# etlundquist/robot-ebert

Measured on AMD Instinct MI355X. Metric: queries/sec + top-K index match, 1M×d=1536 batch=4096, at 1/2/4/8 MI355X, higher is better.
Workload: dtype f64

## Files before the change

include/ebert.h:

```cpp
#ifndef EBERT_H_
#define EBERT_H_

#include <stddef.h>
#include <stdint.h>

#ifdef __cplusplus
extern "C" {
#endif

#define EBT_OK 0
#define EBT_EINVAL (-1)
#define EBT_EHIP (-2)
#define EBT_ENOMEM (-3)
#define EBT_EUNSUPPORTED (-4)

#define EBT_F32 0
#define EBT_BF16 1
#define EBT_F16 2
#define EBT_F64 3

int ebt_version(void);

const char* ebt_last_error(void);

// ... 58 lines not shown
size_t ebt_sort_exclusions_bytes(int64_t B, int64_t nnz);
int ebt_sort_exclusions(const int64_t* off, const int64_t* rows_in, int64_t* rows_out, int64_t B,
                        int64_t nnz, void* workspace, size_t ws_bytes, void* stream);

int ebt_merge_topk(const double* scores, const int64_t* rows, int32_t R, int64_t B, int32_t k,
                   double* out_scores, int64_t* out_rows, void* stream);

int64_t ebt_shard_list_width(int32_t k, int32_t world);
int64_t ebt_shard_sample_tiles(int64_t n_global, int32_t world, int64_t B_pad);
int64_t ebt_shard_pack_cap(int64_t B, int32_t k, int32_t world, int64_t n_global);
size_t ebt_shard_pack_bytes(int64_t B, int64_t cap);
int ebt_shard_pack(const double* scores, const int64_t* rows, int64_t B, int32_t k,
                   const double* t_floor, int64_t cap, void* send, void* stream);
int ebt_merge_packed(const void* recv, int32_t R, int64_t B, int32_t k, int64_t cap,
                     double* out_scores, int64_t* out_rows, int32_t* incomplete, void* stream);

int ebt_screen_exact(const double* q64, int64_t B, int32_t d, const void* cat, int dtype,
                     int64_t ld, const double* gnorm64, int64_t n_rows, float* scores,
                     int64_t ld_scores, void* stream);

#define EBT_FLAG_NO_FUSE 1
#define EBT_FLAG_EXACT 2
#define EBT_FLAG_THETA 4
#define EBT_EXACT_EPS 1.1920928955078125e-07f
int ebt_cosine_topk_plan(int64_t B, int64_t B_pad, int64_t n_rows, int32_t kprime,
                         int64_t chunk_rows, int flags, int64_t* head_rows, int64_t* cap,
                         int64_t* chunk, int32_t* fused);
int ebt_cosine_topk_spec_plan(int64_t B, int64_t B_pad, int64_t n_rows, int32_t kprime,
                              int flags, int64_t* sample_tiles, int64_t* tile_stride,
                              int32_t* rank, double* hits);
int64_t ebt_cosine_topk_spec_lead(int64_t B, int64_t B_pad, int64_t n_rows, int32_t kprime,
                                  int flags);
int ebt_spec_lead(int on);
size_t ebt_cosine_topk_workspace(int64_t B, int64_t B_pad, int64_t n_rows, int32_t kprime,
                                 int64_t chunk_rows, int flags);

int ebt_cosine_topk_prepared(const double* q64, const void* qimg, const float* qscale, const float* eps,
                    int64_t B, int64_t B_pad, const void* cat, int dtype, int64_t ld,
                    const double* gnorm64, const void* cimg, const float* cscale, int img_dtype,
                    int32_t ld_img, int64_t n_rows, int32_t d, int32_t d_pad, int64_t row_offset,
                    const int64_t* excl_off, const int64_t* excl_rows, int32_t k, int32_t kprime,
                    int64_t chunk_rows, int flags, void* workspace, size_t ws_bytes,
                    double* out_scores, int64_t* out_rows, int32_t* certified, void* timer,
                    void* stream);

typedef struct ebt_catalog {
  const void* data;
  int32_t dtype, d;
  int64_t n, ld, row_offset;
  double* gnorm64;
  float* inv32;
  const void* image;
  const float* cscale;
  int32_t img_dtype, ld_img, d_pad, native;
  float u_cat;
} ebt_catalog;

size_t ebt_catalog_state_bytes(const void* data, int dtype, int64_t n, int32_t d, int64_t ld);
int ebt_catalog_init(ebt_catalog* cat, const void* data, int dtype, int64_t n, int32_t d,
                     int64_t ld, int64_t row_offset, void* state, size_t state_bytes,
                     void* stream);

int ebt_catalog_init_reserved(ebt_catalog* cat, const void* data, int dtype, int64_t n,
                              int64_t n_cap, int32_t d, int64_t ld, int64_t row_offset,
                              void* state, size_t state_bytes, void* stream);

// ... 338 lines not shown
```

robot_ebert_amd/_lib.py:

```python
from __future__ import annotations

import ctypes
import os
import threading
from typing import Optional

import torch

_HERE = os.path.dirname(os.path.abspath(__file__))
LIB_PATH = os.environ.get("EBERT_LIB", os.path.join(_HERE, "libebert.so"))

EBT_F32, EBT_BF16, EBT_F16, EBT_F64 = 0, 1, 2, 3
DTYPE_CODE = {torch.float32: EBT_F32, torch.bfloat16: EBT_BF16, torch.float16: EBT_F16,
              torch.float64: EBT_F64}
STAGES = {"gemm": 0, "mask": 1, "select": 2, "merge_select": 3, "rescore": 4, "gemm_filter": 5,
          "prep": 6, "shard_merge": 7, "collective_wait": 8, "small": 9}
EBT_FLAG_NO_FUSE = 1
EBT_FLAG_EXACT = 2
EBT_FLAG_THETA = 4
EBT_FLAG_LIKED_CHECKED = 8
EBT_FILTER_SLOTS_MAX = 128
EBT_EXPLAIN_M_MAX = 64
EBT_MMR_POOL_MAX = 512
EBT_INTEREST_MAX = 8
# ... 186 lines not shown
    "ebt_cosine_sample_lead": ([_VP, _VP, _I64, _VP, _VP, _INT, _I32, _I64, _I32, _I64, _I64,
                                _VP, _I64, _I64, _VP, _I64, _VP, _VP], _INT),
    "ebt_cosine_screen_at_lead": ([_VP, _VP, _VP, _VP, _I64, _I64, _VP, _INT, _I64, _VP, _VP,
                                   _VP, _INT, _I32, _I64, _I32, _I32, _I64, _VP, _VP, _I32,
                                   _I32, _I64, _INT, _VP, ctypes.c_size_t, _VP, _VP, _VP, _VP,
                                   _VP, ctypes.c_double, _I64, _VP, _I64, _VP, _VP], _INT),
    "ebt_pool_kth": ([_VP, _I64, _I64, _I64, _I32, _I32, _VP, _VP], _INT),
    "ebt_union_floor": ([_VP, _I32, _I64, _I32, _I32, _VP, _VP], _INT),
    "ebt_certify_cut": ([_VP, _VP, _VP, _VP, _VP, _I64, _VP], _INT),
    "ebt_rescore_owned": ([_VP, _I64, _I32, _VP, _INT, _I64, _VP, _I64, _I64, _VP, _VP, _I32,
                           _I32, _VP, _VP, _VP], _INT),
    "ebt_finalize_topk": ([_VP, _VP, _VP, _I64, _I32, _I32, _I64, _VP, _VP, _VP, _VP, _VP, _VP],
                          _INT),
    "ebt_merge_hits": ([_VP, _VP, _I64, _I32, _I32, _VP, _I64, _I32, _VP, _I64, _I64, _I64, _VP, _VP, _VP,
                        _VP], _INT),
    "ebt_mask_excluded": ([_VP, _I64, _I64, _I64, _I64, _VP, _VP, _VP], _INT),
    "ebt_select_topk": ([_VP, _VP, _I64, _I64, _I64, _I64, _I32, _I32, _VP, _VP, _I64, _VP],
                        _INT),
    "ebt_rescore": ([_VP, _I64, _I32, _VP, _INT, _I64, _VP, _I64, _VP, _VP, _I32, _I32, _I64, _VP,
                     _VP, _VP, _VP, _VP, _VP, _VP], _INT),
    "ebt_rescore_form": ([_INT], _INT),
    "ebt_wave_sum_check": ([_VP, _I64, _VP, _VP, _VP], _INT),
    "ebt_sort_exclusions_bytes": ([_I64, _I64], _SZ),
    "ebt_sort_exclusions": ([_VP, _VP, _VP, _I64, _I64, _VP, _SZ, _VP], _INT),
    "ebt_merge_topk": ([_VP, _VP, _I32, _I64, _I32, _VP, _VP, _VP], _INT),
    "ebt_screen_exact": ([_VP, _I64, _I32, _VP, _INT, _I64, _VP, _I64, _VP, _I64, _VP], _INT),
    "ebt_cosine_topk_workspace": ([_I64, _I64, _I64, _I32, _I64, _INT], _SZ),
    "ebt_cosine_topk_plan": ([_I64, _I64, _I64, _I32, _I64, _INT, ctypes.POINTER(_I64),
                              ctypes.POINTER(_I64), ctypes.POINTER(_I64),
                              ctypes.POINTER(ctypes.c_int32)], _INT),
    "ebt_cosine_topk_spec_plan": ([_I64, _I64, _I64, _I32, _INT, ctypes.POINTER(_I64),
                                   ctypes.POINTER(_I64), ctypes.POINTER(ctypes.c_int32),
                                   ctypes.POINTER(ctypes.c_double)], _INT),
    "ebt_cosine_topk_prepared": ([_VP, _VP, _VP, _VP, _I64, _I64, _VP, _INT, _I64, _VP, _VP, _VP, _INT,
                         _I32, _I64, _I32, _I32, _I64, _VP, _VP, _I32, _I32, _I64, _INT, _VP, _SZ,
                         _VP, _VP, _VP, _VP, _VP], _INT),
    "ebt_als_gram": ([_VP, _I64, _I32, _VP, _VP], _INT),
    "ebt_als_solve": ([_VP, _VP, _I32, _I64, _VP, _VP, _VP, _F32, _F32, _VP, _VP], _INT),
    "ebt_timer_create": ([], _VP),
    "ebt_timer_destroy": ([_VP], None),
    "ebt_timer_reset": ([_VP], _INT),
    "ebt_timer_set_mask": ([_VP, ctypes.c_uint32], _INT),
    "ebt_timer_query": ([_VP, _INT, ctypes.POINTER(ctypes.c_double), ctypes.POINTER(_I64)], _INT),
    "ebt_timer_begin": ([_VP, _INT, _VP], _INT),
    "ebt_timer_end": ([_VP, _INT, _VP], _INT),
    "ebt_timer_count_rows": ([_VP, _INT], _INT),
    "ebt_timer_rows": ([_VP, ctypes.POINTER(_I64)], _INT),
}

_lib: Optional[ctypes.CDLL] = None
_lock = threading.Lock()


def load() -> ctypes.CDLL:
    global _lib
    if _lib is not None:
        return _lib
    with _lock:
        if _lib is None:
            if not os.path.exists(LIB_PATH):
                raise EbertError(
                    f"{LIB_PATH} not found: build it with `python -c 'import __graft_entry__ as g; "
                    "g.build()'` (make -C robot_ebert_amd/csrc)")
            try:
                lib = ctypes.CDLL(LIB_PATH)
            except OSError as e:
# ... 94 lines not shown
```

robot_ebert_amd/csrc/api.hip:

```cpp
#include <atomic>
#include <cstdarg>
#include <cstdlib>
#include <cstdio>
#include <cstring>
#include <mutex>
#include <vector>

#include "common.h"
#include "internal.h"

namespace ebt {

static thread_local char g_err[512] = "";

void set_error(const char* fmt, ...) {
  va_list ap;
  va_start(ap, fmt);
  vsnprintf(g_err, sizeof(g_err), fmt, ap);
  va_end(ap);
}

int hip_check(hipError_t e, const char* what) {
  if (e == hipSuccess) return EBT_OK;
  set_error("%s: %s", what, hipGetErrorString(e));
// ... 374 lines not shown
  if (selects && L.segs > 1) o = align_up(o + (size_t)B * L.segs * kprime * 4);
  L.off_segi = o;
  if (selects && L.segs > 1) o = align_up(o + (size_t)B * L.segs * kprime * 8);
  L.off_chv = o;
  if (selects && L.n_chunks > 1) o = align_up(o + (size_t)B * L.n_chunks * kprime * 4);
  L.off_chi = o;
  if (selects && L.n_chunks > 1) o = align_up(o + (size_t)B * L.n_chunks * kprime * 8);
  L.off_fv = o;
  o = align_up(o + (size_t)B * kprime * 4);
  L.off_fi = o;
  o = align_up(o + (size_t)B * kprime * 8);
  if (L.fused) {
    L.off_cand = o;
    o = align_up(o + (size_t)B_pad * L.ld_cand * 8);
    L.off_counts = o;
    o = align_up(o + (size_t)B_pad * L.ld_counts);
    L.off_thr = o;
    o = align_up(o + (size_t)B_pad * 4);
    L.off_ovf = o;
    o = align_up(o + (size_t)B_pad * 4);
  }
  L.off_eps = o;
  if (flags & EBT_FLAG_EXACT) o = align_up(o + (size_t)B_pad * 4);
  if (L.spec) {
    L.off_tspec = o;
    o = align_up(o + (size_t)B_pad * 4);
  }
  L.off_lead = o;
  if (L.ld_lead) o = align_up(o + (size_t)B_pad * L.ld_lead * 4);
  L.bytes = o;
  return L;
}

static int head_topk(const PipeArgs& a, const WsLayout& L, char* ws, int64_t r0, int64_t nrows,
                     float* dv_final, int64_t* di_final, int64_t ld_final, void* timer,
                     hipStream_t st) {
  const QueryOps& q = a.q;
  const CatOps& c = a.c;
  const int64_t B = q.B, row_offset = c.row_offset;
  const int32_t kprime = a.kprime;
  const bool exact = a.flags & EBT_FLAG_EXACT;
  float* S = (float*)(ws + L.off_s);
  float* segv = (float*)(ws + L.off_segv);
  int64_t* segi = (int64_t*)(ws + L.off_segi);
  float* chv = (float*)(ws + L.off_chv);
  int64_t* chi = (int64_t*)(ws + L.off_chi);
  const int64_t n_chunks = ceil_div(nrows, L.chunk);
  int rc;
  for (int64_t ch = 0; ch < n_chunks; ++ch) {
    const int64_t c0 = r0 + ch * L.chunk;
    const int64_t nc = (r0 + nrows - c0) < L.chunk ? (r0 + nrows - c0) : L.chunk;
    {
      StageScope s(timer, EBT_STAGE_GEMM, st);
      if (exact) {
        rc = screen_exact(q.q64, B, c.d, (const char*)c.cat + c0 * c.ld * dtype_size(c.dtype),
                          c.dtype, c.ld,
                          c.gnorm64 + c0, nc, S, L.ld_s, st);
      } else {
        rc = screen_gemm(q.qimg, q.B_pad, (const char*)c.cimg + c0 * c.ld_img * 2, nc, c.d_pad,
                         c.ld_img, c.img_dtype, q.qscale, c.cscale ? c.cscale + c0 : nullptr, S,
                         L.ld_s, st);
      }
    }
    if (rc) return rc;
    if (a.excl.off || a.allow) {
      StageScope s(timer, EBT_STAGE_MASK, st);
// ... 14 lines not shown
      } else {
        rc = select_topk(S, nullptr, L.ld_s, B, nc, c0, kprime, L.segs, segv, segi,
                         (int64_t)L.segs * kprime, st);
        if (!rc)
          rc = select_topk(segv, segi, (int64_t)L.segs * kprime, B, (int64_t)L.segs * kprime, 0,
                           kprime, 1, dv, di, ld_d, st);
      }
    }
    if (rc) return rc;
  }
  if (n_chunks > 1) {
    StageScope s(timer, EBT_STAGE_MERGE_SELECT, st);
    rc = select_topk(chv, chi, n_chunks * kprime, B, n_chunks * kprime, 0, kprime, 1, dv_final,
                     di_final, ld_final, st);
    if (rc) return rc;
  }
  return EBT_OK;
}

int rescore_sharded(const double* q64, int64_t B, const CatOps& c, const CandList& l, int32_t k,
                    const float* eps, const double* t_floor, double* out_s, int64_t* out_r,
                    int32_t* certified, RescoreExtras x, void* timer, hipStream_t st) {
  StageScope sc(timer, EBT_STAGE_RESCORE, st);
  x.gathered = timer_rows(timer, st);
  return rescore(q64, B, c, l, k, eps, t_floor, out_s, out_r, certified, x, st);
}

}

using namespace ebt;

extern "C" {

int ebt_version(void) { return 1200; }

const char* ebt_last_error(void) { return g_err; }

int ebt_row_norms(const void* x, int dtype, int64_t n, int32_t d, int64_t ld, double* gnorm64,
                  float* inv32, void* stream) {
  return row_norms(x, dtype, n, d, ld, gnorm64, inv32, (hipStream_t)stream);
}

int ebt_screen_image(const void* x, int dtype, int64_t n, int32_t d, int64_t ld,
                     const double* gnorm64, int normalize, int img_dtype, void* img,
                     int32_t ld_img, void* stream) {
  return screen_image(x, dtype, n, d, ld, gnorm64, normalize, img_dtype, img, ld_img,
                      (hipStream_t)stream);
}

int ebt_query_dense(const void* q, int dtype, int64_t B, int32_t d, int64_t ldq, double* q64,
                    void* stream) {
  return query_dense(q, dtype, B, d, ldq, q64, (hipStream_t)stream);
}

int ebt_query_liked_sum(const void* cat, int dtype, int32_t d, int64_t ld,
                        const double* gnorm64_cat, int64_t B, const int64_t* liked_off,
                        const int64_t* liked_rows, double* q64, void* stream) {
  return query_liked_sum(cat, dtype, d, ld, gnorm64_cat, B, liked_off, liked_rows, q64,
                         (hipStream_t)stream, 0, 0);
}

int ebt_query_liked_wsum(const void* cat, int dtype, int32_t d, int64_t ld,
                         const double* gnorm64_cat, int64_t B, const int64_t* liked_off,
                         const int64_t* liked_rows, const double* liked_w, double* q64,
                         void* stream) {
  return query_liked_wsum(cat, dtype, d, ld, gnorm64_cat, B, liked_off, liked_rows, liked_w, q64,
                          (hipStream_t)stream, 0, 0);
// ... 116 lines not shown
    return EBT_EINVAL;
  }
  const WsLayout L = ws_layout(B, B_pad, n_rows, kprime, chunk_rows, flags);
  *head_rows = L.head;
  *cap = L.fused ? L.seg_max : 0;
  *chunk = L.chunk;
  *fused = L.fused ? 1 : 0;
  return EBT_OK;
}

int ebt_cosine_topk_spec_plan(int64_t B, int64_t B_pad, int64_t n_rows, int32_t kprime,
                              int flags, int64_t* sample_tiles, int64_t* tile_stride,
                              int32_t* rank, double* hits) {
  if (B < 0 || B_pad < B || n_rows < 1 || kprime < 1 || !sample_tiles || !tile_stride || !rank ||
      !hits) {
    set_error("ebt_cosine_topk_spec_plan: bad arguments");
    return EBT_EINVAL;
  }
  const WsLayout L = ws_layout(B, B_pad, n_rows, kprime, 1024, flags);
  *sample_tiles = L.spec ? L.spec_tiles : 0;
  *tile_stride = L.spec ? L.spec_stride : 0;
  *rank = L.spec ? L.spec_j : 0;
  *hits = L.spec ? L.spec_hits : 0.0;
  return EBT_OK;
}

int64_t ebt_cosine_topk_spec_lead(int64_t B, int64_t B_pad, int64_t n_rows, int32_t kprime,
                                  int flags) {
  if (B < 0 || B_pad < B || n_rows < 1 || kprime < 1) return -1;
  const WsLayout L = ws_layout(B, B_pad, n_rows, kprime, 1024, flags);
  return L.spec ? L.spec_lead : 0;
}

int ebt_spec_lead(int on) {
  if (on < 0) return spec_lead_flag().load();
  return spec_lead_flag().exchange(on != 0 ? 1 : 0);
}

}

namespace ebt {
namespace {

struct ScreenOut {
  float* fv;
  int64_t* fi;
  const float* eps;
  const int* ovf;
  const float* theta;
};

}

static int check_pipe(const PipeArgs& a, const char* who) {
  const QueryOps& q = a.q;
  const CatOps& c = a.c;
  const bool exact = a.flags & EBT_FLAG_EXACT;
  if (!q.q64 || (!exact && (!q.qimg || !q.qscale || !q.eps || !c.cimg)) || !c.cat ||
      !c.gnorm64) {
    set_error("%s: null pointer", who);
    return EBT_EINVAL;
  }
  if (q.B < 1 || q.B_pad < q.B || q.B_pad % 128 != 0 || c.n_rows < 1 || c.d < 1 ||
      c.d_pad < c.d || c.d_pad % 64 != 0 || c.ld_img < c.d_pad || a.k < 1 || a.kprime < a.k ||
      a.kprime > 4096 || a.kprime % 4 != 0 || a.chunk_rows < 128 || a.chunk_rows % 128 != 0 ||
      ((a.excl.off == nullptr) != (a.excl.rows == nullptr))) {
    set_error("%s: bad arguments (B=%lld B_pad=%lld n=%lld d=%d d_pad=%d k=%d kprime=%d "
              "chunk=%lld)", who, (long long)q.B, (long long)q.B_pad, (long long)c.n_rows, c.d,
              c.d_pad, a.k, a.kprime, (long long)a.chunk_rows);
    return EBT_EINVAL;
  }
  return EBT_OK;
}

static int filter_screen(const PipeArgs& a, int64_t r0, int64_t seg, const float* thr,
                         const HitSlots& h, int* ovf, void* timer, hipStream_t st) {
  const QueryOps& q = a.q;
  const CatOps& c = a.c;
  const int64_t part = filter_split_rows(q.B_pad, seg);
  const int64_t step = part > 0 ? part : seg;
  for (int64_t p0 = 0; p0 < seg; p0 += step) {
    const int64_t nr = seg - p0 < step ? seg - p0 : step;
    const int64_t r = r0 + p0;
    const HitSlots hp = from_group(h, p0 / 256);
    KernelStage s(timer, EBT_STAGE_GEMM_FILTER, st);
    const int rc = screen_gemm_filter(q.qimg, q.B_pad, (const char*)c.cimg + r * c.ld_img * 2, nr,
                                      c.d_pad, c.ld_img, c.img_dtype, q.qscale,
                                      c.cscale ? c.cscale + r : nullptr, thr, hp.cand, hp.ld_cand,
                                      hp.slots, hp.counts, hp.ld_counts, ovf, r, st);
    if (rc) return rc;
  }
  return EBT_OK;
}

static int run_screen_spec(const PipeArgs& a, const WsLayout& L, char* ws, float* fv,
                           int64_t* fi, void* timer, hipStream_t st) {
  int rc;
  const QueryOps& q = a.q;
  const CatOps& c = a.c;
  const int64_t B = q.B, B_pad = q.B_pad, n_rows = c.n_rows;
  const int32_t k = a.k, kprime = a.kprime;
  float* thr = (float*)(ws + L.off_thr);
  int* ovf = (int*)(ws + L.off_ovf);
  float* pooled = (float*)(ws + L.off_s);
  float* tspec = (float*)(ws + L.off_tspec);
  const int64_t m = L.head;
  const bool given = a.theta != nullptr || a.gsamp != nullptr;
  const double spec_hits = given ? (a.hits > 0.0 ? a.hits : 1.0) : L.spec_hits;
  const double per_group = spec_hits * (double)L.group_rows / (double)n_rows;
  const double n_cells = (double)B * (double)ceil_div(n_rows, L.group_rows);
  int slots = 8;
  while (slots < EBT_FILTER_SLOTS_MAX &&
         (slots < 4.0 * per_group + 4.0 || n_cells * poisson_tail(1.5 * per_group, slots) > 1e-3))
    slots *= 2;
  const HitSlots h{(uint64_t*)(ws + L.off_cand), L.ld_cand, slots, (uint8_t*)(ws + L.off_counts),
                   L.ld_counts};
  float* own_lead = (float*)(ws + L.off_lead);
  const LeadIn li = given ? a.lead : LeadIn{own_lead, L.ld_lead, L.spec_lead};
  const int64_t lead = li.tiles;
  if (lead > 0 && (lead * slots > L.ld_cand || lead > L.ld_counts || L.group_rows != 256)) {
    set_error("run_screen_spec: the lead does not fit the hit slots");
    return EBT_EINVAL;
  }
  if (given) {
    if (a.gsamp)
      rc = pool_kth(a.gsamp, a.gs_G, B, B_pad, a.gs_G, a.gs_j, tspec, fv, fi, kprime, ovf, li, h,
                    a.gs, st);
    else
      rc = spec_given_init(a.theta, B, B_pad, tspec, fv, fi, kprime, ovf, li, h, st);
    if (rc) return rc;
  } else {
    {
      StageScope s(timer, EBT_STAGE_GEMM, st);
      rc = screen_gemm_pool(q.qimg, B_pad, c.cimg, m, c.d_pad, c.ld_img, c.img_dtype, q.qscale,
                            c.cscale, 256 * L.spec_stride, pooled, L.ld_s, st, lead, own_lead,
                            L.ld_lead);
    }
    if (rc) return rc;
    {
      StageScope s(timer, EBT_STAGE_SELECT, st);
      rc = pool_kth(pooled, L.ld_s, B, B_pad, (int)(m / 64), L.spec_j, tspec, fv, fi, kprime, ovf,
                    li, h, {}, st);
    }
    if (rc) return rc;
  }
  const bool wave = merge_wave_fits(kprime);
  int64_t seg_cap = L.ld_cand / slots;
  const int64_t max_groups = wave ? merge_wave_max_groups() : merge_block_max_groups(kprime);
  seg_cap = seg_cap < max_groups ? seg_cap : max_groups;
  seg_cap *= L.group_rows;
  const double cap = (double)(wave ? merge_wave_capacity() : merge_block_capacity(kprime));
  double f_spread = 2.5;
  if (!given && L.spec_j > 0) {
    const double target = 1e-2 / (double)(B > 0 ? B : 1);
    double x = (double)L.spec_j;
    while (x < 8.0 * L.spec_j) {
      double pmf = exp(-x), cdf = pmf;
      for (int i = 1; i < L.spec_j; ++i) {
        pmf *= x / i;
        cdf += pmf;
      }
      if (cdf <= target) break;
      x += 0.25;
    }
    f_spread = x / (double)L.spec_j;
    f_spread = f_spread < 2.5 ? 2.5 : f_spread;
  }
  int64_t r0 = 256 * lead;
  bool first = true, verified = false, thr_raised = false;
  while (r0 < n_rows) {
    const int64_t g0 = first ? lead : 0;
    const int64_t cap_rows = seg_cap - g0 * L.group_rows;
    const double room = (cap - kprime) / f_spread;
    const double kept = 0.5 * ((double)k + (double)kprime);
    double rate = spec_hits / (double)n_rows;
    if (!first && kept / (double)r0 < rate) rate = kept / (double)r0;
    int64_t seg = (int64_t)(room / (rate > 1e-12 ? rate : 1e-12));
    seg = (seg + 255) / 256 * 256;
    if (L.round_rows > 0 && seg >= L.round_rows) seg = seg / L.round_rows * L.round_rows;
    seg = seg < 256 ? 256 : seg;
    const int64_t cap_r = L.round_rows > 0 && cap_rows >= L.round_rows
                              ? cap_rows / L.round_rows * L.round_rows : cap_rows;
    seg = seg < cap_r ? seg : cap_r;
    if (!first && n_rows - r0 - seg < seg / 2) seg = n_rows - r0;
    if (seg > cap_rows) seg = cap_rows;
    if (seg > n_rows - r0) seg = n_rows - r0;
    if (seg < 1) {
      set_error("run_screen_spec: no room for a segment");
      return EBT_EINVAL;
    }
    const float* t = tspec;
    if (!first) {
      if (!thr_raised) {
        rc = spec_threshold(fv, kprime, B, B_pad, k, q.eps, tspec, thr, ovf, 0, st);
        if (rc) return rc;
      }
      t = thr;
    }
    rc = filter_screen(a, r0, seg, t, from_group(h, g0), ovf, timer, st);
    if (rc) return rc;
    const bool fuse_verify = wave && !given && r0 + seg == n_rows;
    verified |= fuse_verify;
    const int64_t groups = g0 + ceil_div(seg, L.group_rows);
    const bool last = r0 + seg == n_rows;
    thr_raised = wave && !last;
    {
      StageScope s(timer, EBT_STAGE_MERGE_SELECT, st);
      if (wave) {
        WaveMergeOpts o{};
        if (fuse_verify) o.verify = {tspec, q.eps};
        if (last && a.floor_out) o.floor = {a.floor_out, a.floor_w, q.eps};
        if (thr_raised) o.raise = {thr, tspec, q.eps, B_pad};
        rc = merge_segment_wave(fv, fi, B, kprime, k, h, groups, c.row_offset, a.excl, ovf, st, o);
      } else {
        rc = merge_segment(fv, fi, B, kprime, h, groups, c.row_offset, a.excl, ovf, st,
                           rate * (double)(seg + g0 * L.group_rows));
      }
    }
    if (rc) return rc;
    r0 += seg;
    first = false;
  }
  if (given || verified) return EBT_OK;
  return spec_threshold(fv, kprime, B, B_pad, k, q.eps, tspec, nullptr, ovf, 1, st);
}

static int run_screen(const PipeArgs& a, const WsLayout& L, char* ws, float* fv, int64_t* fi,
                      void* timer, hipStream_t st, ScreenOut* so) {
  int rc;
  const QueryOps& q = a.q;
  const CatOps& c = a.c;
  so->eps = q.eps;
  so->ovf = nullptr;
  const int64_t B = q.B, B_pad = q.B_pad, n_rows = c.n_rows, row_offset = c.row_offset;
  const int32_t k = a.k, kprime = a.kprime;
  if (a.flags & EBT_FLAG_EXACT) {
    float* xeps = (float*)(ws + L.off_eps);
    const float e = EBT_EXACT_EPS;
    uint32_t bits;
    memcpy(&bits, &e, 4);
    rc = hip_check(hipMemsetD32Async((hipDeviceptr_t)xeps, (int)bits, (size_t)B, st),
                   "hipMemsetD32Async");
    if (rc) return rc;
    so->eps = xeps;
    return head_topk(a, L, ws, 0, n_rows, fv, fi, kprime, timer, st);
  }
  if (!L.fused) return head_topk(a, L, ws, 0, n_rows, fv, fi, kprime, timer, st);
  float* thr = (float*)(ws + L.off_thr);
// ... 427 lines not shown
```

robot_ebert_amd/csrc/internal.h:

```cpp
#pragma once

#include "common.h"

namespace ebt {

struct QueryOps {
  const double* q64;
  const void* qimg;
  const float *qscale, *eps;
  int64_t B, B_pad;
};
struct CatOps {
  const void* cat; int dtype; int64_t ld; const double* gnorm64;
  const void* cimg; const float* cscale; int img_dtype; int32_t ld_img;
  int64_t n_rows; int32_t d, d_pad; int64_t row_offset;
};
inline CatOps cat_ops(const ebt_catalog& c) {
  return {c.data, c.dtype, c.ld, c.gnorm64, c.image, c.cscale, c.img_dtype, c.ld_img, c.n, c.d,
          c.d_pad, c.row_offset};
}
struct ExclCsr { const int64_t *off, *rows; };
struct HitSlots {
  uint64_t* cand; int64_t ld_cand; int slots;
  uint8_t* counts; int64_t ld_counts;
// ... 26 lines not shown
struct RescoreExtras {
  const int* ovf; const float* theta; ExclCsr excl;
  const ShardPackOut* pack; unsigned long long* gathered;
};

int64_t shard_lead_room(int64_t B_pad, int64_t n_rows, int64_t sample_tiles);
int64_t shard_lead_tiles(int64_t B_pad, int64_t n_rows, int64_t sample_tiles);
int rescore_sharded(const double* q64, int64_t B, const CatOps& c, const CandList& l, int32_t k,
                    const float* eps, const double* t_floor, double* out_s, int64_t* out_r,
                    int32_t* certified, RescoreExtras x, void* timer, hipStream_t st);
int topk_prepared(const PipeArgs& a, void* workspace, size_t ws_bytes, double* out_scores,
                  int64_t* out_rows, int32_t* certified, void* timer, hipStream_t st);
int screen_export(const PipeArgs& a, void* workspace, size_t ws_bytes, float* list_vals,
                  int64_t* list_rows, int32_t* ovf_out, float* eps_out, void* timer,
                  hipStream_t st);
int screen_at_local(const PipeArgs& a, void* workspace, size_t ws_bytes, float* list_vals,
                    int64_t* list_rows, const float** theta_dev, const int** ovf_dev,
                    const float** eps_dev, void* timer, hipStream_t st);

int64_t gemm_cus();
int screen_gemm(const void* qimg, int64_t B_pad, const void* cimg, int64_t n_rows, int32_t d_pad,
                int32_t ld_img, int img_dtype, const float* qscale, const float* cscale,
                float* scores, int64_t ld_scores, hipStream_t stream, int64_t cstride = 0);
int screen_gemm_pool(const void* qimg, int64_t B_pad, const void* cimg, int64_t n_rows,
                     int32_t d_pad, int32_t ld_img, int img_dtype, const float* qscale,
                     const float* cscale, int64_t cstride, float* pooled, int64_t ld_pooled,
                     hipStream_t stream, int64_t lead, float* lead_scores, int64_t ld_lead);
int64_t filter_group_rows(int64_t B_pad);
int screen_gemm_filter(const void* qimg, int64_t B_pad, const void* cimg, int64_t n_rows,
                       int32_t d_pad, int32_t ld_img, int img_dtype, const float* qscale,
                       const float* cscale, const float* thr, uint64_t* cand, int64_t ld_cand,
                       int slots, uint8_t* counts, int64_t ld_counts, int* ovf, int64_t idx_base,
                       hipStream_t stream);
int64_t filter_split_rows(int64_t B_pad, int64_t n_rows);

int select_topk(const float* vals, const int64_t* idx, int64_t ld, int64_t B, int64_t n,
                int64_t idx_base, int32_t kprime, int32_t segs, float* out_vals, int64_t* out_idx,
                int64_t ld_out, hipStream_t stream);
int merge_segment(float* fv, int64_t* fi, int64_t B, int kprime, const HitSlots& h,
                  int64_t n_groups, int64_t row_offset, const ExclCsr& excl, int* ovf,
                  hipStream_t st, double expect_hits = 0.0);
bool merge_wave_fits(int kprime);
int merge_block_capacity(int kprime);
int64_t merge_block_max_groups(int kprime);
int64_t merge_wave_max_groups();
int merge_wave_capacity();
int merge_segment_wave(float* fv, int64_t* fi, int64_t B, int kprime, int k, const HitSlots& h,
                       int64_t n_groups, int64_t row_offset, const ExclCsr& excl, int* ovf,
                       hipStream_t st, const WaveMergeOpts& o = {});
int pilot_topk(const float* S, int64_t ld_s, int64_t B, int n, int64_t idx_base, int kprime, int k,
               float* fv, int64_t* fi, hipStream_t st);
int kth_threshold(const float* vals, int64_t ld, int64_t B, int64_t B_pad, int k, const float* eps,
                  float* thr, hipStream_t st);
int pool_kth(const float* pool, int64_t ld, int64_t B, int64_t B_pad, int G, int j, float* thr,
             float* fv, int64_t* fi, int kprime, int* ovf, const LeadIn& lead, const HitSlots& h,
             const GatheredSamples& gs, hipStream_t st);
int spec_given_init(const float* theta, int64_t B, int64_t B_pad, float* tspec, float* fv,
                    int64_t* fi, int kprime, int* ovf, const LeadIn& lead, const HitSlots& h,
                    hipStream_t st);
int spec_threshold(const float* vals, int64_t ld, int64_t B, int64_t B_pad, int k,
                   const float* eps, const float* thr_spec, float* thr, int* ovf, int mode,
                   hipStream_t st);

int row_norms(const void* x, int dtype, int64_t n, int32_t d, int64_t ld, double* gnorm,
              float* inv32, hipStream_t st);
int screen_image(const void* x, int dtype, int64_t n, int32_t d, int64_t ld, const double* gnorm,
                 int normalize, int img_dtype, void* img, int32_t ld_img, hipStream_t st,
// ... 55 lines not shown
```

robot_ebert_amd/csrc/screen_gemm.hip:

```cpp
#include <hip/hip_ext.h>

#include <atomic>
#include <cstdlib>
#include <type_traits>

#include "common.h"
#include "internal.h"

namespace ebt {

constexpr int GBM = 128;
constexpr int GBN = 128;
constexpr int GBK = 64;
constexpr int GTHREADS = 256;
constexpr int GTILE_BYTES = GBM * GBK * 2;
constexpr int GSTAGE_BYTES = 2 * GTILE_BYTES;
constexpr int GLDS_BYTES = 2 * GSTAGE_BYTES;
constexpr int GGROUP_C = 8;

typedef __attribute__((address_space(3))) void lds_void;
typedef __attribute__((address_space(1))) const void gbl_cvoid;

__device__ __forceinline__ void stage_operand(const uint16_t* __restrict__ X, int64_t ldx,
                                              int64_t row0, int64_t last_row, int k0,
// ... 1333 lines not shown
  return v;
}
static int64_t filter_tiles_per_wg() { return filter_tpw_flag().load(std::memory_order_relaxed); }

int screen_gemm_filter(const void* qimg, int64_t B_pad, const void* cimg, int64_t n_rows,
                       int32_t d_pad, int32_t ld_img, int img_dtype, const float* qscale,
                       const float* cscale, const float* thr, uint64_t* cand, int64_t ld_cand,
                       int slots, uint8_t* counts, int64_t ld_counts, int* ovf, int64_t idx_base,
                       hipStream_t stream) {
  int rc = check_gemm_args("ebt_screen_filter", qimg, B_pad, cimg, n_rows, d_pad, ld_img,
                           img_dtype, qscale, cscale);
  if (rc) return rc;
  const int64_t groups = ceil_div(n_rows, filter_group_rows(B_pad));
  if (!thr || !cand || !counts || !ovf || slots < 1 || slots > EBT_FILTER_SLOTS_MAX ||
      ld_counts < groups || ld_cand < groups * slots || idx_base < 0 ||
      idx_base + n_rows > 0xffffffffLL) {
    set_error("ebt_screen_filter: bad candidate buffers (groups=%lld ld_cand=%lld ld_counts=%lld)",
              (long long)groups, (long long)ld_cand, (long long)ld_counts);
    return EBT_EINVAL;
  }
  EpiArgs e{};
  e.thr = thr;
  e.cand = cand;
  e.ld_cand = ld_cand;
  e.counts = counts;
  e.ld_counts = ld_counts;
  e.ovf = ovf;
  e.idx_base = idx_base;
  e.slots = slots;
  return launch_gemm<EPI_FILTER>(qimg, B_pad, cimg, n_rows, d_pad, ld_img, img_dtype, qscale,
                                 cscale, e, stream);
}

int64_t filter_split_rows(int64_t B_pad, int64_t n_rows) {
  const int64_t tpw = filter_tiles_per_wg();
  const int64_t qt = B_pad / QP_TILE;
  if (tpw <= 0 || B_pad % QP_TILE != 0 || qt < 1 || n_cus() % qt != 0) return 0;
  const int64_t round_rows = (n_cus() / qt) * QP_TILE;
  const int64_t cap_rows = tpw * round_rows;
  if (n_rows <= cap_rows + cap_rows / 2) return 0;
  const int64_t parts = (n_rows + cap_rows - 1) / cap_rows;
  return (n_rows / parts + round_rows - 1) / round_rows * round_rows;
}

}

extern "C" int64_t ebt_filter_split(int64_t tiles_per_workgroup) {
  if (tiles_per_workgroup < 0) return ebt::filter_tpw_flag().load();
  return ebt::filter_tpw_flag().exchange(tiles_per_workgroup);
}
```

robot_ebert_amd/search.py:

```python
from __future__ import annotations

import os
from dataclasses import dataclass
from typing import Optional, Sequence, Tuple, Union

import numpy as np
import torch

from . import _lib
from ._lib import DTYPE_CODE, EbertError, call, ptr, region, require_cuda, stream_of
from .catalog import Catalog

KPRIME_MAX = 4096
QUERY_PREP_MAX_D = 4096
MERGE_WAVE_KMAX = 512
DEFAULT_SCORE_BUDGET = int(os.environ.get("EBT_SCORE_BUDGET", str(4 << 30)))


def _round_up(v: int, m: int) -> int:
    return (v + m - 1) // m * m


def pad_batch(B: int) -> int:
    B = max(B, 1)
# ... 256 lines not shown


def default_kprime(catalog: Catalog, k: int) -> int:
    kp = k + max(16, k // 4) if catalog.native else max(2 * k, k + 32)
    return min(_round_up(kp, 8), KPRIME_MAX)


def _clamp_kprime(catalog: Catalog, k_eff: int, kprime: Optional[int] = None) -> int:
    kp = kprime or default_kprime(catalog, k_eff)
    return max(_round_up(k_eff, 4), min(_round_up(kp, 4), _round_up(catalog.n, 4), KPRIME_MAX))


def _chunk_rows(catalog: Catalog, B_pad: int, budget: int) -> int:
    rows = budget // (4 * B_pad)
    rows = max(128, rows // 128 * 128)
    return min(rows, _round_up(catalog.n, 128))


def plan(catalog: Catalog, B: int, k: int, kprime: Optional[int] = None,
         chunk_rows: Optional[int] = None, fuse: bool = True) -> dict:
    import ctypes
    B_pad = pad_batch(B)
    k_eff = min(k, catalog.n)
    kp = _clamp_kprime(catalog, k_eff, kprime)
    chunk = chunk_rows or _chunk_rows(catalog, B_pad, DEFAULT_SCORE_BUDGET)
    h, c, ch = ctypes.c_int64(), ctypes.c_int64(), ctypes.c_int64()
    f = ctypes.c_int32()
    call("ebt_cosine_topk_plan", B, B_pad, catalog.n, kp, chunk,
         0 if fuse else _lib.EBT_FLAG_NO_FUSE, ctypes.byref(h), ctypes.byref(c), ctypes.byref(ch),
         ctypes.byref(f))
    out = {"kprime": kp, "B_pad": B_pad, "fused": bool(f.value), "head_rows": h.value,
           "segment_rows_max": c.value, "chunk_rows": ch.value}
    out["spec"] = spec_plan(B, catalog.n, kp, fuse)
    return out


def spec_plan(B: int, n: int, kprime: int, fuse: bool = True) -> Optional[dict]:
    import ctypes
    t, st, h = ctypes.c_int64(), ctypes.c_int64(), ctypes.c_double()
    j = ctypes.c_int32()
    call("ebt_cosine_topk_spec_plan", B, pad_batch(B), n, kprime,
         0 if fuse else _lib.EBT_FLAG_NO_FUSE, ctypes.byref(t), ctypes.byref(st), ctypes.byref(j),
         ctypes.byref(h))
    if t.value == 0:
        return None
    lead = int(_lib.load().ebt_cosine_topk_spec_lead(B, pad_batch(B), n, kprime,
                                                     0 if fuse else _lib.EBT_FLAG_NO_FUSE))
    return {"tiles": t.value, "stride": st.value, "rank": j.value, "hits": round(h.value, 1),
            "lead": lead}


def _pipe_operands(catalog: Catalog, qb: QueryBatch, exclude, k: int, kprime: int, chunk: int,
                   flags: int) -> tuple:
    eo, er = exclude if exclude is not None else (None, None)
    return (ptr(qb.q64), ptr(qb.qimg), ptr(qb.qscale), ptr(qb.eps), qb.B, qb.B_pad,
            ptr(catalog.data), catalog.dtype_code, catalog.ld, ptr(catalog.gnorm),
            ptr(catalog.image), ptr(catalog.cscale), catalog.img_dtype, catalog.ld_img, catalog.n,
            catalog.d, catalog.d_pad, catalog.row_offset, ptr(eo), ptr(er), k, kprime, chunk,
            flags)


def _pipe_buffers(catalog: Catalog, qb: QueryBatch, kprime: int, chunk_rows: Optional[int],
                  flags: int, workspace: Optional[torch.Tensor] = None):
    chunk = chunk_rows or _chunk_rows(catalog, qb.B_pad, DEFAULT_SCORE_BUDGET)
    need = _lib.load().ebt_cosine_topk_workspace(qb.B, qb.B_pad, catalog.n, kprime, chunk, flags)
    if need == 0:
        raise EbertError("invalid workspace request")
    if workspace is None or workspace.numel() < need:
        workspace = torch.empty(need, dtype=torch.uint8, device=catalog.device)
    return chunk, workspace


def run_pipeline(catalog: Catalog, qb: QueryBatch, k: int, kprime: int,
                 exclude: Optional[Tuple[torch.Tensor, torch.Tensor]] = None,
                 chunk_rows: Optional[int] = None, timer: Optional[_lib.Timer] = None,
                 workspace: Optional[torch.Tensor] = None, flags: int = 0, allow=None):
    import ctypes
    from .allow import resolve_allow
    dev = catalog.device
    B = qb.B
    ra = resolve_allow(allow, B, dev)
    if ra is not None and not flags & _lib.EBT_FLAG_EXACT:
# ... 580 lines not shown
```

Before: 412,300.

## Size later speculative segments with a raised spread and adaptive slot counts

Moves speculative-screen segment planning into shared helpers. Later segments, once the running threshold has risen, use a smaller spread factor derived from a negative-binomial tail bound, and a reduced per-group hit-slot count. The filter split now balances rounds evenly across launches instead of using a fixed step. A planning API exposes the schedule. The intent is larger and fewer segments, which means fewer filter and merge launches and less candidate memory. The cost is a looser statistical margin that could raise overflow risk.

```diff
diff --git a/include/ebert.h b/include/ebert.h
--- a/include/ebert.h
+++ b/include/ebert.h
@@ -114,6 +114,11 @@
 int64_t ebt_cosine_topk_spec_lead(int64_t B, int64_t B_pad, int64_t n_rows, int32_t kprime,
                                   int flags);
 int ebt_spec_lead(int on);
+int ebt_cosine_topk_spec_segments(int64_t B, int64_t B_pad, int64_t n_rows, int32_t k,
+                                  int32_t kprime, int flags, double given_hits,
+                                  int64_t given_lead, int32_t max_segments, int64_t* seg_rows,
+                                  double* seg_hits, double* seg_spread, int64_t* seg_parts,
+                                  int32_t* n_segments, double* room);
 size_t ebt_cosine_topk_workspace(int64_t B, int64_t B_pad, int64_t n_rows, int32_t kprime,
                                  int64_t chunk_rows, int flags);
 
diff --git a/robot_ebert_amd/_lib.py b/robot_ebert_amd/_lib.py
--- a/robot_ebert_amd/_lib.py
+++ b/robot_ebert_amd/_lib.py
@@ -242,6 +242,12 @@
     "ebt_cosine_topk_spec_plan": ([_I64, _I64, _I64, _I32, _INT, ctypes.POINTER(_I64),
                                    ctypes.POINTER(_I64), ctypes.POINTER(ctypes.c_int32),
                                    ctypes.POINTER(ctypes.c_double)], _INT),
+    "ebt_cosine_topk_spec_segments": ([_I64, _I64, _I64, _I32, _I32, _INT, ctypes.c_double, _I64,
+                                       _I32, ctypes.POINTER(_I64),
+                                       ctypes.POINTER(ctypes.c_double),
+                                       ctypes.POINTER(ctypes.c_double), ctypes.POINTER(_I64),
+                                       ctypes.POINTER(ctypes.c_int32),
+                                       ctypes.POINTER(ctypes.c_double)], _INT),
     "ebt_cosine_topk_prepared": ([_VP, _VP, _VP, _VP, _I64, _I64, _VP, _INT, _I64, _VP, _VP, _VP, _INT,
                          _I32, _I64, _I32, _I32, _I64, _VP, _VP, _I32, _I32, _I64, _INT, _VP, _SZ,
                          _VP, _VP, _VP, _VP, _VP], _INT),
diff --git a/robot_ebert_amd/csrc/api.hip b/robot_ebert_amd/csrc/api.hip
--- a/robot_ebert_amd/csrc/api.hip
+++ b/robot_ebert_amd/csrc/api.hip
@@ -430,6 +430,125 @@
   return L;
 }
 
+
+static double negbin_tail(int j, double mu, int m) {
+  const double p = mu / ((double)j + mu);
+  double pmf = pow((double)j / ((double)j + mu), (double)j), cdf = pmf;
+  for (int x = 0; x < m; ++x) {
+    pmf *= ((double)x + (double)j) / ((double)x + 1.0) * p;
+    cdf += pmf;
+  }
+  return 1.0 - cdf;
+}
+
+constexpr double SPEC_RAISED_SPREAD = 2.0;
+constexpr double SPEC_RATE_ERR = 1.25;
+static double spec_raised_spread(int k, double room, double target) {
+  static thread_local struct { int k; double room, target, s; } memo = {0, 0.0, 0.0, 0.0};
+  if (memo.k == k && memo.room == room && memo.target == target) return memo.s;
+  double s = 1.0;
+  while (s < 8.0 && negbin_tail(k, room / s, (int)room) > target) s += 0.01;
+  memo = {k, room, target, s * SPEC_RATE_ERR};
+  return memo.s;
+}
+
+static int spec_slots(const WsLayout& L, int64_t B, int64_t n_rows, double spec_hits) {
+  const double per_group = spec_hits * (double)L.group_rows / (double)n_rows;
+  const double n_cells = (double)B * (double)ceil_div(n_rows, L.group_rows);
+  int slots = 8;
+  while (slots < EBT_FILTER_SLOTS_MAX &&
+         (slots < 4.0 * per_group + 4.0 || n_cells * poisson_tail(1.5 * per_group, slots) > 1e-3))
+    slots *= 2;
+  return slots;
+}
+
+struct SpecSegs {
+  int64_t B, n_rows, lead, max_groups;
+  int slots;
+  double spec_hits, kept, cap_room, f_spread, f_raised, f_join;
+  bool wave, raised_slots;
+};
+
+static SpecSegs spec_segs(const WsLayout& L, int64_t B, int64_t n_rows, int32_t k,
+                          int32_t kprime, bool given, double spec_hits, int64_t lead, int slots) {
+  SpecSegs p{};
+  p.B = B;
+  p.n_rows = n_rows;
+  p.lead = lead;
+  p.slots = slots;
+  p.spec_hits = spec_hits;
+  p.wave = merge_wave_fits(kprime);
+  p.max_groups = p.wave ? merge_wave_max_groups() : merge_block_max_groups(kprime);
+  const double cap = (double)(p.wave ? merge_wave_capacity() : merge_block_capacity(kprime));
+  p.cap_room = cap - kprime;
+  p.kept = 0.5 * ((double)k + (double)kprime);
+  p.f_spread = 2.5;
+  const double target = 1e-2 / (double)(B > 0 ? B : 1);
+  if (!given && L.spec_j > 0) {
+    double x = (double)L.spec_j;
+    while (x < 8.0 * L.spec_j) {
+      double pmf = exp(-x), cdf = pmf;
+      for (int i = 1; i < L.spec_j; ++i) {
+        pmf *= x / i;
+        cdf += pmf;
+      }
+      if (cdf <= target) break;
+      x += 0.25;
+    }
+    p.f_spread = x / (double)L.spec_j;
+    p.f_spread = p.f_spread < 2.5 ? 2.5 : p.f_spread;
+  }
+  p.f_raised = p.f_spread;
+  if (!given && p.wave && p.cap_room >= 1.0) {
+    const double f = spec_raised_spread(k, p.cap_room, target);
+    p.f_join = f < p.f_spread ? f : p.f_spread;
+    p.f_raised = p.f_join < SPEC_RAISED_SPREAD ? SPEC_RAISED_SPREAD : p.f_join;
+    p.f_raised = p.f_raised < p.f_spread ? p.f_raised : p.f_spread;
+    p.raised_slots = true;
+  }
+  return p;
+}
+
+static int64_t spec_next_segment(const WsLayout& L, const SpecSegs& p, int64_t r0, bool first,
+                                 double* rate_out, double* spread_out, int* slots_out) {
+  const int64_t g0 = first ? p.lead : 0;
+  double rate = p.spec_hits / (double)p.n_rows;
+  double spread = p.f_spread;
+  int slots = p.slots;
+  bool raised = false;
+  if (!first && p.kept / (double)r0 < rate) {
+    rate = p.kept / (double)r0;
+    spread = p.f_raised;
+    if (p.raised_slots) {
+      raised = true;
+      slots = spec_slots(L, p.B, p.n_rows, rate * (double)p.n_rows);
+      slots = slots < p.slots ? slots : p.slots;
+    }
+  }
+  int64_t seg_cap = L.ld_cand / slots;
+  seg_cap = (seg_cap < p.max_groups ? seg_cap : p.max_groups) * L.group_rows;
+  const int64_t cap_rows = seg_cap - g0 * L.group_rows;
+  *slots_out = slots;
+  const double room = p.cap_room / spread;
+  int64_t seg = (int64_t)(room / (rate > 1e-12 ? rate : 1e-12));
+  seg = (seg + 255) / 256 * 256;
+  if (L.round_rows > 0 && seg >= L.round_rows) seg = seg / L.round_rows * L.round_rows;
+  seg = seg < 256 ? 256 : seg;
+  const int64_t cap_r = L.round_rows > 0 && cap_rows >= L.round_rows
+                            ? cap_rows / L.round_rows * L.round_rows : cap_rows;
+  seg = seg < cap_r ? seg : cap_r;
+  if (!first && p.n_rows - r0 > seg && p.n_rows - r0 - seg < seg / 2 &&
+      (!raised || rate * (double)(p.n_rows - r0) * p.f_join <= p.cap_room)) {
+    seg = p.n_rows - r0;
+    if (raised && seg <= cap_rows) spread = p.f_join;
+  }
+  if (seg > cap_rows) seg = cap_rows;
+  if (seg > p.n_rows - r0) seg = p.n_rows - r0;
+  *rate_out = rate;
+  *spread_out = spread;
+  return seg < 1 ? 0 : seg;
+}
+
 static int head_topk(const PipeArgs& a, const WsLayout& L, char* ws, int64_t r0, int64_t nrows,
                      float* dv_final, int64_t* di_final, int64_t ld_final, void* timer,
                      hipStream_t st) {
@@ -510,7 +629,7 @@
 
 extern "C" {
 
-int ebt_version(void) { return 1200; }
+int ebt_version(void) { return 1201; }
 
 const char* ebt_last_error(void) { return g_err; }
 
@@ -693,6 +812,58 @@
   return L.spec ? L.spec_lead : 0;
 }
 
+int ebt_cosine_topk_spec_segments(int64_t B, int64_t B_pad, int64_t n_rows, int32_t k,
+                                  int32_t kprime, int flags, double given_hits,
+                                  int64_t given_lead, int32_t max_segments, int64_t* seg_rows,
+                                  double* seg_hits, double* seg_spread, int64_t* seg_parts,
+                                  int32_t* n_segments, double* room) {
+  if (B < 1 || B_pad < B || n_rows < 1 || k < 1 || kprime < k || max_segments < 0 ||
+      given_lead < 0 || (max_segments > 0 && (!seg_rows || !seg_hits || !seg_spread)) ||
+      !n_segments || !room) {
+    set_error("ebt_cosine_topk_spec_segments: bad arguments");
+    return EBT_EINVAL;
+  }
+  const bool given = given_hits >= 0.0;
+  const WsLayout L =
+      ws_layout(B, B_pad, n_rows, kprime, 1024, given ? flags | EBT_FLAG_THETA : flags);
+  *n_segments = 0;
+  *room = 0.0;
+  if (!L.spec) return EBT_OK;
+  const double spec_hits = given ? (given_hits > 0.0 ? given_hits : 1.0) : L.spec_hits;
+  const int64_t lead = given ? given_lead : L.spec_lead;
+  if (256 * lead > n_rows) {
+    set_error("ebt_cosine_topk_spec_segments: the lead exceeds the catalog");
+    return EBT_EINVAL;
+  }
+  const int slots = spec_slots(L, B, n_rows, spec_hits);
+  const SpecSegs segs = spec_segs(L, B, n_rows, k, kprime, given, spec_hits, lead, slots);
+  *room = segs.cap_room;
+  int32_t n = 0;
+  bool first = true;
+  for (int64_t r0 = 256 * lead; r0 < n_rows; first = false) {
+    double rate, spread;
+    int seg_slots;
+    const int64_t seg = spec_next_segment(L, segs, r0, first, &rate, &spread, &seg_slots);
+    if (seg < 1) {
+      set_error("ebt_cosine_topk_spec_segments: no room for a segment");
+      return EBT_EINVAL;
+    }
+    if (n < max_segments) {
+      seg_rows[n] = seg;
+      seg_hits[n] = rate * (double)(seg + (first ? lead * L.group_rows : 0));
+      seg_spread[n] = spread;
+      if (seg_parts) {
+        int64_t round_rows = 0;
+        seg_parts[n] = filter_split_parts(B_pad, seg, &round_rows);
+      }
+    }
+    ++n;
+    r0 += seg;
+  }
+  *n_segments = n;
+  return EBT_OK;
+}
+
 int ebt_spec_lead(int on) {
   if (on < 0) return spec_lead_flag().load();
   return spec_lead_flag().exchange(on != 0 ? 1 : 0);
@@ -738,10 +909,10 @@
                          const HitSlots& h, int* ovf, void* timer, hipStream_t st) {
   const QueryOps& q = a.q;
   const CatOps& c = a.c;
-  const int64_t part = filter_split_rows(q.B_pad, seg);
-  const int64_t step = part > 0 ? part : seg;
-  for (int64_t p0 = 0; p0 < seg; p0 += step) {
-    const int64_t nr = seg - p0 < step ? seg - p0 : step;
+  int64_t round_rows = 0, p0 = 0;
+  const int64_t parts = filter_split_parts(q.B_pad, seg, &round_rows);
+  for (int64_t p = 0; p < parts; ++p) {
+    const int64_t nr = filter_part_rows(seg, round_rows, parts, p, &p0);
     const int64_t r = r0 + p0;
     const HitSlots hp = from_group(h, p0 / 256);
     KernelStage s(timer, EBT_STAGE_GEMM_FILTER, st);
@@ -768,12 +939,7 @@
   const int64_t m = L.head;
   const bool given = a.theta != nullptr || a.gsamp != nullptr;
   const double spec_hits = given ? (a.hits > 0.0 ? a.hits : 1.0) : L.spec_hits;
-  const double per_group = spec_hits * (double)L.group_rows / (double)n_rows;
-  const double n_cells = (double)B * (double)ceil_div(n_rows, L.group_rows);
-  int slots = 8;
-  while (slots < EBT_FILTER_SLOTS_MAX &&
-         (slots < 4.0 * per_group + 4.0 || n_cells * poisson_tail(1.5 * per_group, slots) > 1e-3))
-    slots *= 2;
+  const int slots = spec_slots(L, B, n_rows, spec_hits);
   const HitSlots h{(uint64_t*)(ws + L.off_cand), L.ld_cand, slots, (uint8_t*)(ws + L.off_counts),
                    L.ld_counts};
   float* own_lead = (float*)(ws + L.off_lead);
@@ -806,50 +972,19 @@
     if (rc) return rc;
   }
   const bool wave = merge_wave_fits(kprime);
-  int64_t seg_cap = L.ld_cand / slots;
-  const int64_t max_groups = wave ? merge_wave_max_groups() : merge_block_max_groups(kprime);
-  seg_cap = seg_cap < max_groups ? seg_cap : max_groups;
-  seg_cap *= L.group_rows;
-  const double cap = (double)(wave ? merge_wave_capacity() : merge_block_capacity(kprime));
-  double f_spread = 2.5;
-  if (!given && L.spec_j > 0) {
-    const double target = 1e-2 / (double)(B > 0 ? B : 1);
-    double x = (double)L.spec_j;
-    while (x < 8.0 * L.spec_j) {
-      double pmf = exp(-x), cdf = pmf;
-      for (int i = 1; i < L.spec_j; ++i) {
-        pmf *= x / i;
-        cdf += pmf;
-      }
-      if (cdf <= target) break;
-      x += 0.25;
-    }
-    f_spread = x / (double)L.spec_j;
-    f_spread = f_spread < 2.5 ? 2.5 : f_spread;
-  }
+  const SpecSegs segs = spec_segs(L, B, n_rows, k, kprime, given, spec_hits, lead, slots);
   int64_t r0 = 256 * lead;
   bool first = true, verified = false, thr_raised = false;
   while (r0 < n_rows) {
     const int64_t g0 = first ? lead : 0;
-    const int64_t cap_rows = seg_cap - g0 * L.group_rows;
-    const double room = (cap - kprime) / f_spread;
-    const double kept = 0.5 * ((double)k + (double)kprime);
-    double rate = spec_hits / (double)n_rows;
-    if (!first && kept / (double)r0 < rate) rate = kept / (double)r0;
-    int64_t seg = (int64_t)(room / (rate > 1e-12 ? rate : 1e-12));
-    seg = (seg + 255) / 256 * 256;
-    if (L.round_rows > 0 && seg >= L.round_rows) seg = seg / L.round_rows * L.round_rows;
-    seg = seg < 256 ? 256 : seg;
-    const int64_t cap_r = L.round_rows > 0 && cap_rows >= L.round_rows
-                              ? cap_rows / L.round_rows * L.round_rows : cap_rows;
-    seg = seg < cap_r ? seg : cap_r;
-    if (!first && n_rows - r0 - seg < seg / 2) seg = n_rows - r0;
-    if (seg > cap_rows) seg = cap_rows;
-    if (seg > n_rows - r0) seg = n_rows - r0;
+    double rate, spread;
+    int seg_slots;
+    const int64_t seg = spec_next_segment(L, segs, r0, first, &rate, &spread, &seg_slots);
     if (seg < 1) {
       set_error("run_screen_spec: no room for a segment");
       return EBT_EINVAL;
     }
+    const HitSlots hs{h.cand, h.ld_cand, seg_slots, h.counts, h.ld_counts};
     const float* t = tspec;
     if (!first) {
       if (!thr_raised) {
@@ -858,7 +993,7 @@
       }
       t = thr;
     }
-    rc = filter_screen(a, r0, seg, t, from_group(h, g0), ovf, timer, st);
+    rc = filter_screen(a, r0, seg, t, from_group(hs, g0), ovf, timer, st);
     if (rc) return rc;
     const bool fuse_verify = wave && !given && r0 + seg == n_rows;
     verified |= fuse_verify;
@@ -872,9 +1007,9 @@
         if (fuse_verify) o.verify = {tspec, q.eps};
         if (last && a.floor_out) o.floor = {a.floor_out, a.floor_w, q.eps};
         if (thr_raised) o.raise = {thr, tspec, q.eps, B_pad};
-        rc = merge_segment_wave(fv, fi, B, kprime, k, h, groups, c.row_offset, a.excl, ovf, st, o);
+        rc = merge_segment_wave(fv, fi, B, kprime, k, hs, groups, c.row_offset, a.excl, ovf, st, o);
       } else {
-        rc = merge_segment(fv, fi, B, kprime, h, groups, c.row_offset, a.excl, ovf, st,
+        rc = merge_segment(fv, fi, B, kprime, hs, groups, c.row_offset, a.excl, ovf, st,
                            rate * (double)(seg + g0 * L.group_rows));
       }
     }
diff --git a/robot_ebert_amd/csrc/internal.h b/robot_ebert_amd/csrc/internal.h
--- a/robot_ebert_amd/csrc/internal.h
+++ b/robot_ebert_amd/csrc/internal.h
@@ -82,7 +82,9 @@
                        const float* cscale, const float* thr, uint64_t* cand, int64_t ld_cand,
                        int slots, uint8_t* counts, int64_t ld_counts, int* ovf, int64_t idx_base,
                        hipStream_t stream);
-int64_t filter_split_rows(int64_t B_pad, int64_t n_rows);
+int64_t filter_split_parts(int64_t B_pad, int64_t n_rows, int64_t* round_rows);
+int64_t filter_part_rows(int64_t n_rows, int64_t round_rows, int64_t parts, int64_t p,
+                         int64_t* row0);
 
 int select_topk(const float* vals, const int64_t* idx, int64_t ld, int64_t B, int64_t n,
                 int64_t idx_base, int32_t kprime, int32_t segs, float* out_vals, int64_t* out_idx,
diff --git a/robot_ebert_amd/csrc/screen_gemm.hip b/robot_ebert_amd/csrc/screen_gemm.hip
--- a/robot_ebert_amd/csrc/screen_gemm.hip
+++ b/robot_ebert_amd/csrc/screen_gemm.hip
@@ -1389,15 +1389,30 @@
                                  cscale, e, stream);
 }
 
-int64_t filter_split_rows(int64_t B_pad, int64_t n_rows) {
+int64_t filter_split_parts(int64_t B_pad, int64_t n_rows, int64_t* round_rows) {
   const int64_t tpw = filter_tiles_per_wg();
   const int64_t qt = B_pad / QP_TILE;
-  if (tpw <= 0 || B_pad % QP_TILE != 0 || qt < 1 || n_cus() % qt != 0) return 0;
-  const int64_t round_rows = (n_cus() / qt) * QP_TILE;
-  const int64_t cap_rows = tpw * round_rows;
-  if (n_rows <= cap_rows + cap_rows / 2) return 0;
-  const int64_t parts = (n_rows + cap_rows - 1) / cap_rows;
-  return (n_rows / parts + round_rows - 1) / round_rows * round_rows;
+  *round_rows = 0;
+  if (tpw <= 0 || B_pad % QP_TILE != 0 || qt < 1 || n_cus() % qt != 0) return 1;
+  *round_rows = (n_cus() / qt) * QP_TILE;
+  const int64_t cap_rows = tpw * *round_rows;
+  if (n_rows <= cap_rows + cap_rows / 2) return 1;
+  return (n_rows + cap_rows - 1) / cap_rows;
+}
+
+int64_t filter_part_rows(int64_t n_rows, int64_t round_rows, int64_t parts, int64_t p,
+                         int64_t* row0) {
+  if (parts <= 1 || round_rows <= 0) {
+    *row0 = 0;
+    return n_rows;
+  }
+  const int64_t rounds = (n_rows + round_rows - 1) / round_rows;
+  const int64_t base = rounds / parts, extra = rounds % parts;
+  const int64_t first = p * base + (p < extra ? p : extra);
+  const int64_t count = base + (p < extra ? 1 : 0);
+  *row0 = first * round_rows;
+  const int64_t end = (first + count) * round_rows;
+  return (end < n_rows && p + 1 < parts ? end : n_rows) - *row0;
 }
 
 }
diff --git a/robot_ebert_amd/search.py b/robot_ebert_amd/search.py
--- a/robot_ebert_amd/search.py
+++ b/robot_ebert_amd/search.py
@@ -312,6 +312,8 @@
     out = {"kprime": kp, "B_pad": B_pad, "fused": bool(f.value), "head_rows": h.value,
            "segment_rows_max": c.value, "chunk_rows": ch.value}
     out["spec"] = spec_plan(B, catalog.n, kp, fuse)
+    if out["spec"] is not None:
+        out["spec"]["segments"] = spec_segments(B, catalog.n, k_eff, kp, fuse)["segments"]
     return out
 
 
@@ -328,6 +330,25 @@
                                                      0 if fuse else _lib.EBT_FLAG_NO_FUSE))
     return {"tiles": t.value, "stride": st.value, "rank": j.value, "hits": round(h.value, 1),
             "lead": lead}
+
+
+def spec_segments(B: int, n: int, k: int, kprime: int, fuse: bool = True,
+                  given_hits: Optional[float] = None, given_lead: int = 0) -> dict:
+    import ctypes
+    cap = 64
+    while True:
+        rows, parts = (ctypes.c_int64 * cap)(), (ctypes.c_int64 * cap)()
+        hits, spread = (ctypes.c_double * cap)(), (ctypes.c_double * cap)()
+        ns, room = ctypes.c_int32(), ctypes.c_double()
+        call("ebt_cosine_topk_spec_segments", B, pad_batch(B), n, k, kprime,
+             0 if fuse else _lib.EBT_FLAG_NO_FUSE, -1.0 if given_hits is None else given_hits,
+             given_lead, cap, rows, hits, spread, parts, ctypes.byref(ns), ctypes.byref(room))
+        if ns.value <= cap:
+            break
+        cap = ns.value
+    return {"room": room.value,
+            "segments": [{"rows": rows[i], "hits": hits[i], "spread": spread[i],
+                          "launches": parts[i]} for i in range(ns.value)]}
 
 
 def _pipe_operands(catalog: Catalog, qb: QueryBatch, exclude, k: int, kprime: int, chunk: int,
```

Result: no change. 412,300, median of 3 (-0.0%).
